# kai0511/insider

Measured on AMD Instinct MI355X. Metric: outer-iterations/sec (masked INSIDER fit, 10000 x 50000, K=30), higher is better.
Workload: dtype f64

## Files before the change

insider_amd/csrc/insider_col_factored.hpp:

```cpp
#pragma once

namespace insider {

constexpr int CP_MAXSTEPS = 8;
constexpr int CP_MAXCELLS = 4096;

struct ColFacArgs {
    int p, K, c;
    size_t plane;
    const uint32_t *grp[CF_MAXC];
    const uint16_t *slev[CF_MAXC];
    int L[CF_MAXC + 1], off[CF_MAXC + 1];
    int nlater[CF_MAXC + 1];
    int later_plane[CF_MAXC][CF_MAXC];
    int tab_skip_lo, tab_skip_n;
    int tab_rows;
    const double *Astack;
    const double *Qheld;
    const double *RtR;
    const double *yy_all, *yy_train;
    double *stat;
    const uint8_t *cnt;
    int cnt_stride, cnt_off[CF_MAXC + 1], nsteps;
    const float *hn;
    int hn_stride, hn_off[CF_MAXC + 1];
    const double *zt;
    int zt_stride, zt_off[CF_MAXC + 1];
    int m, SLcat;
    int pos_cov[CF_MAXC];
};

template <int NB, bool PREMASKED = false>
__device__ __forceinline__ void cf_store(d4 (&acc)[NB][NB], double *tr, const ColFacArgs &a, int j, int lane,
                                         const double *rtr, const double (&qh)[NB], double ss)
{
    constexpr int KP = Geo<NB>::KP;
    const int g4 = lane >> 4, c16 = lane & 15;
    double *out = a.stat + (size_t)j * Geo<NB>::STAT;
    int blk = 0;
#pragma unroll
    for (int bi = 0; bi < NB; ++bi)
#pragma unroll
        for (int bj = 0; bj <= bi; ++bj, ++blk) {
#pragma unroll
            for (int r = 0; r < 4; ++r) tr[(g4 + 4 * r) * 17 + c16] = acc[bj][bi][r];
            wave_sync();
            d4 res;
#pragma unroll
            for (int r = 0; r < 4; ++r) {
                const int ra = 16 * bi + g4 + 4 * r, cb = 16 * bj + c16;
                res[r] = acc[bi][bj][r] + tr[c16 * 17 + g4 + 4 * r];
                if constexpr (PREMASKED) res[r] = rtr[ra * KP + cb] - res[r];
// ... 204 lines not shown
            for (int s = 0; s < 4; ++s)
                if (l0 + 4 * s < Lo) {
#pragma unroll
                    for (int bi = 0; bi < NB; ++bi)
#pragma unroll
                        for (int bj = 0; bj < NB; ++bj)
                            acc[bi][bj] = __builtin_amdgcn_mfma_f64_16x16x4f64(cur.av[s][bi], P[bj][s], acc[bi][bj], 0, 0, 0);
                }
        };
        PairBlk<NB> b0, b1;
        fetch(0, b0);
        for (int l0 = 0; l0 < Lo; l0 += 32) {
            if (l0 + 16 < Lo) fetch(l0 + 16, b1);
            compute(l0, b0);
            if (l0 + 16 < Lo) {
                if (l0 + 32 < Lo) fetch(l0 + 32, b0);
                compute(l0 + 16, b1);
            }
        }
    }
    cf_store<NB, true>(acc, tr, a, j, lane, rtr, qh, ss);
}

template <int NB, int WPB, int MAXS, bool ZC = false>
__global__ void __launch_bounds__(WPB * 64) k_col_paircnt4(ColFacArgs a, unsigned *__restrict__ ticket, unsigned ticket_base, int npart, int cap)
{
    static_assert(NB <= 2, "accumulators of the 4x4x4 form");
    constexpr int KP = Geo<NB>::KP;
    extern __shared__ double s_c4[];
    const int w = __builtin_amdgcn_readfirstlane(threadIdx.x >> 6), lane = threadIdx.x & 63;
    double *tr = s_c4 + (size_t)w * 16 * 17;
    double *rtr = s_c4 + (size_t)WPB * 16 * 17;
    double *tabs = rtr + KP * KP;
    double *rows = tabs + 4 * a.nsteps * KP;
    const int npos = a.c + (ZC ? 1 : 0);
    for (int i = threadIdx.x; i < KP * KP; i += WPB * 64) rtr[i] = (i / KP < a.K && i % KP < a.K) ? a.RtR[i] : 0.0;
    for (int i = threadIdx.x; i < 4 * a.nsteps * KP; i += WPB * 64) {
        const int r = i / KP, k = i % KP;
        const int q = r < a.tab_skip_lo ? r : r + a.tab_skip_n;
        tabs[i] = r < a.tab_rows ? a.Astack[(size_t)q * KP + k] : 0.0;
    }
    {
        int pb4 = 0;
        for (int t = 0; t < npos; ++t) {
            const int nq = (a.L[t] + 3) >> 2;
            const double *At = a.Astack + (size_t)a.off[t] * KP;
            for (int i = threadIdx.x; i < 4 * nq * KP; i += WPB * 64) {
                const int l = i / KP, k = i % KP;
                rows[((size_t)(pb4 + (l >> 2)) * NB + (k >> 4)) * 64 + (l & 3) * 16 + (k & 15)] = At[i];
            }
            pb4 += nq;
        }
        for (int i = threadIdx.x; i < 4 * KP; i += WPB * 64) rows[(size_t)pb4 * NB * 64 + i] = 0.0;
    }
    __syncthreads();
    const int g4 = lane >> 4, c16 = lane & 15;
    constexpr int bpl = MAXS <= 4 ? 4 : 8;
    double tb[MAXS][NB];
#pragma unroll
    for (int s = 0; s < MAXS; ++s)
#pragma unroll
        for (int bb = 0; bb < NB; ++bb) tb[s][bb] = s < a.nsteps ? tabs[(4 * s + g4) * KP + 16 * bb + c16] : 0.0;
    double tbz[NB];
#pragma unroll
    for (int bb = 0; bb < NB; ++bb) tbz[bb] = ZC ? a.Astack[(size_t)(a.SLcat + g4) * KP + 16 * bb + c16] : 0.0;
    const unsigned off_c = (unsigned)lane * (unsigned)bpl, off_h = (unsigned)g4 * 4u;
    const double *rl[4];
#pragma unroll
    for (int x = 0; x < 4; ++x) rl[x] = rows + g4 * 16 + ((c16 + 4 * x) & 15);
    struct Blk {
        uint32_t cw[2];
        float4 hn;
        double z;
    };
    const int part = blockIdx.x % npart;
    unsigned *tk = ticket + 32 * part;
    auto take = [&]() {
        unsigned v = 0;
        if (lane == 0) v = atomicAdd(tk, 1u);
        return (unsigned)__builtin_amdgcn_readfirstlane((int)v) - ticket_base;
    };
    for (unsigned cur = take(), nxt; cur < (unsigned)cap; cur = nxt) {
    nxt = take();
    const int j = (int)cur * npart + part;
    if (j >= a.p) continue;
    double qh[NB];
#pragma unroll
    for (int bb = 0; bb < NB; ++bb) qh[bb] = a.Qheld[(size_t)j * KP + 16 * bb + c16];
    const double ss = a.yy_all[j] - a.yy_train[j];
    double acc[NB][NB][4];
#pragma unroll
    for (int bi = 0; bi < NB; ++bi)
#pragma unroll
        for (int bj = 0; bj < NB; ++bj)
#pragma unroll
            for (int x = 0; x < 4; ++x) acc[bi][bj][x] = 0.0;
    const uint8_t *cj = a.cnt + (size_t)j * a.cnt_stride;
    const float *hj = a.hn + (size_t)j * a.hn_stride;
    const double *zj = ZC ? a.zt + (size_t)j * a.zt_stride : nullptr;
    int pb4 = 0;
    for (int t = 0; t < npos; ++t) {
        const int Lo = a.L[t];
        const bool cross = a.nlater[t] > 0;
        const uint8_t *ct = cj + a.cnt_off[t];
        const float *ht = hj + a.hn_off[t];
        const double *zt = ZC ? zj + a.zt_off[t] : nullptr;
        auto fetch = [&](int l0, Blk &b) {
            if constexpr (ZC) b.z = zt[(size_t)(l0 >> 4) * 64 + lane];
            b.cw[0] = b.cw[1] = 0;
            if (cross) {
                const uint32_t *src = reinterpret_cast<const uint32_t *>(ct + (size_t)(l0 >> 4) * 64 * bpl + off_c);
                b.cw[0] = src[0];
                if (bpl == 8) b.cw[1] = src[1];
            }
            b.hn = *reinterpret_cast<const float4 *>(ht + l0 + off_h);
        };
        const double *rp[4];
#pragma unroll
        for (int x = 0; x < 4; ++x) rp[x] = rl[x] + (size_t)pb4 * NB * 64;
        auto rows_of = [&](int s, double (&av)[4][NB]) {
#pragma unroll
            for (int x = 0; x < 4; ++x)
#pragma unroll
                for (int bi = 0; bi < NB; ++bi) av[x][bi] = rp[x][(s * NB + bi) * 64];
        };
        auto step = [&](const double (&av)[4][NB], double hn, const d4 (&P)[NB], int s) {
            double pr[NB];
#pragma unroll
            for (int bb = 0; bb < NB; ++bb) pr[bb] = fma(hn, av[0][bb], P[bb][s]);
#pragma unroll
            for (int bi = 0; bi < NB; ++bi)
#pragma unroll
                for (int bj = 0; bj < NB; ++bj)
#pragma unroll
                    for (int x = 0; x < 4; ++x)
                        acc[bi][bj][x] = __builtin_amdgcn_mfma_f64_4x4x4f64(av[x][bi], pr[bj], acc[bi][bj][x], 0, 0, 0);
        };
        double avA[4][NB], avB[4][NB];
        auto compute = [&](int l0, const Blk &cur) {
            d4 P[NB];
#pragma unroll
            for (int bb = 0; bb < NB; ++bb) P[bb] = d4{0.0, 0.0, 0.0, 0.0};
            if (cross) {
#pragma unroll
                for (int s = 0; s < MAXS; ++s)
                    if (s < a.nsteps) {
                        const double cv = (double)((cur.cw[s >> 2] >> (8 * (s & 3))) & 0xffu);
#pragma unroll
                        for (int bb = 0; bb < NB; ++bb)
                            P[bb] = __builtin_amdgcn_mfma_f64_16x16x4f64(cv, tb[s][bb], P[bb], 0, 0, 0);
                    }
            }
            if constexpr (ZC) {
#pragma unroll
                for (int bb = 0; bb < NB; ++bb) P[bb] = __builtin_amdgcn_mfma_f64_16x16x4f64(cur.z, tbz[bb], P[bb], 0, 0, 0);
            }
            rows_of(1, avB);
            __builtin_amdgcn_sched_barrier(0);
            step(avA, (double)cur.hn.x, P, 0);
            if (l0 + 4 < Lo) {
                rows_of(2, avA);
            __builtin_amdgcn_sched_barrier(0);
                step(avB, (double)cur.hn.y, P, 1);
                if (l0 + 8 < Lo) {
                    rows_of(3, avB);
// ... 26 lines not shown
        const int b = c16 >> 2, jj = c16 & 3;
        double *out = a.stat + (size_t)j * Geo<NB>::STAT;
        int blk = 0;
#pragma unroll
        for (int bi = 0; bi < NB; ++bi)
#pragma unroll
            for (int bj = 0; bj <= bi; ++bj, ++blk) {
#pragma unroll
                for (int x = 0; x < 4; ++x) tr[(4 * ((b + x) & 3) + g4) * 17 + 4 * b + jj] = acc[bi][bj][x];
                wave_sync();
                d4 res;
#pragma unroll
                for (int r = 0; r < 4; ++r) res[r] = tr[(g4 + 4 * r) * 17 + c16];
                wave_sync();
#pragma unroll
                for (int x = 0; x < 4; ++x) tr[(4 * ((b + x) & 3) + g4) * 17 + 4 * b + jj] = acc[bj][bi][x];
                wave_sync();
#pragma unroll
                for (int r = 0; r < 4; ++r) {
                    const int ra = 16 * bi + g4 + 4 * r, cb = 16 * bj + c16;
                    res[r] = rtr[ra * KP + cb] - (res[r] + tr[c16 * 17 + g4 + 4 * r]);
                }
                wave_sync();
                if (bi == NB - 1 && g4 == 3) {
                    const int col = 16 * bj + c16;
                    res[3] = col < a.K ? qh[bj] : (col == KP - 1 ? ss : 0.0);
                }
#pragma unroll
                for (int r = 0; r < 4; ++r) out[blk * 256 + (g4 + 4 * r) * 16 + c16] = res[r];
            }
    }
    }
}

__global__ void __launch_bounds__(256) k_zt_build(ColFacArgs a, const uint32_t *__restrict__ col_ptr, const int *__restrict__ col_idx,
                                                  const double *__restrict__ col_val, const int *__restrict__ lev,
                                                  const double *__restrict__ Zc, int n, double *__restrict__ zt,
                                                  double *__restrict__ xz , int xz_pitch,
                                                  const double *__restrict__ S_all, double *__restrict__ S_train )
{
    const int w = threadIdx.x >> 6, lane = threadIdx.x & 63;
    const int j = blockIdx.x * 4 + w;
    if (j >= a.p) return;
    const uint32_t eb = col_ptr[j], ee = col_ptr[j + 1];
    double *zo = zt + (size_t)j * a.zt_stride;
    for (int t = 0; t < a.c; ++t) {
        const int *lv = lev + (size_t)a.pos_cov[t] * n;
        for (int l = lane; l < a.L[t]; l += WAVE) {
            double s[4] = {0.0, 0.0, 0.0, 0.0};
            for (uint32_t e = eb; e < ee; ++e) {
                const int i = col_idx[e];
                if (i < n && lv[i] == l) {
#pragma unroll
                    for (int k = 0; k < 4; ++k)
                        if (k < a.m) s[k] += Zc[(size_t)k * n + i];
// ... 216 lines not shown
```

insider_amd/csrc/insider_hip.hip:

```cpp
#include "insider_kernels.hpp"
#include "insider_posthoc.hpp"
#include "insider_vardecomp.hpp"
#include "insider_sampdecomp.hpp"
#include "insider_levelscores.hpp"
#include "insider_factdecomp.hpp"
#include "insider_rescomp.hpp"
#include "insider_outliers.hpp"
#include "insider_neighbors.hpp"
#include "insider_coexpr.hpp"
#include "insider_enrich.hpp"
#include "insider_kmeans.hpp"
#include "insider_tsne.hpp"

#include <rccl/rccl.h>

#include <algorithm>
#include <chrono>
#include <cstdlib>
#include <cmath>
#include <cstdio>
#include <cstring>
#include <limits>
#include <memory>
#include <mutex>
// ... 186 lines not shown
    DevBuf<int> lev, lvl_off_d, members_all, lvl_ptr_all, lvl_count_all;
    std::vector<CovTables> cov;
    CovTables cont;
    DevBuf<double> Zc;
    DevBuf<int> one_count;
    DevBuf<int> ident_members;
    int max_chunks = 0, max_L = 0, max_items = 0;
    DevBuf<double> S, yy_train, yy_all;
    DevBuf<double> Strain;
    DevBuf<double> Sheld;
    double cnt_train = 0, cnt_test = 0;
    bool no_na = false;
    DevBuf<uint32_t> col_ptr, row_ptr;
    DevBuf<int> col_idx, row_idx;
    DevBuf<double> col_val, row_val;
    DevBuf<uint8_t> col_flag;
    uint64_t col_entries = 0, row_entries = 0;
    bool merged = false;
    ColFacArgs cf;
    int cf_pos[CF_MAXC] = {0};
    bool cf_pair_ok = false;
    DevBuf<uint8_t> cf_cnt;
    DevBuf<float> cf_hn;
    DevBuf<double> cf_zt;
    std::vector<CovTables> contm;
    CovTables contm_lists;
    DevBuf<double> cont_cnt;
    bool cont_merged = false;
    std::vector<DevBuf<double>> cont_pair;
    std::shared_ptr<const HostTables> host;
    mutable std::mutex fold_mu;
    mutable std::shared_ptr<const FoldIds> folds;
    std::shared_ptr<const FoldIds> get_folds() const { std::lock_guard<std::mutex> g(fold_mu); return folds; }
    size_t bytes_shared = 0, bytes_own = 0;

    struct Block { int rows, off; };
    int blocks() const { return c + (m > 0 ? 1 : 0); }
    Block block(int b) const { return b < c ? Block{n_levels[b], lvl_off[b]} : Block{m, SLcat}; }

    DataSet() = default;
    DataSet(const DataSet &) = delete;
    DataSet &operator=(const DataSet &) = delete;
    ~DataSet() { (void)hipSetDevice(device); }
};

struct Workspace {
// ... 71 lines not shown
    }
    int synchronize_sides() const
    {
        for (const Stream *s : {&side, &side2, &side3}) HIPCHECK(hipStreamSynchronize(*s));
        return INSIDER_OK;
    }
    void synchronize() const
    {
        for (const Stream *s : {&stream, &side, &side2, &side3}) if (*s) (void)hipStreamSynchronize(*s);
    }
};

struct Options {
    int max_sweeps = 1 << 24, order_mode = 0, profile = 0, verbose = 0, cd_variant = 0, force_allreduce = 0;
    int col_factored = 1;
    int row_counts = 1;
    int row_merged = 1;
    int row_gemm = 1;
    int wg_waves = 1024;
    int row_fused = 1;
    int mm_fast = 1;
    int mm_tiles = 0;
    int col_mfma4 = 1;
    int cd_pairs = 1;
    int list_fine = 1;
    int cd_cold_iters = 3, cd_pass_first = 64, cd_pass_ratio = 4;
    double resid_stage_mb = 256.0;
    double vd_stage_kb = 48.0;
    int sd_slabs = 0;
    int ls_slabs = 0;
    double ls_part_mb = 256.0;
    int glm_slabs = 0;
    int rc_slabs = 0;
};

struct PostWs {
    DevBuf<double> Ast, U, cp, part, stats, stage, gpart, gram, cpart, gsum, L, dinv, outs;
    DevBuf<int> nz, ints, info;
    DevBuf<double> vin, vtab, vrec;
    DevBuf<double> spart, srec;
    DevBuf<double> lcand, ltab, lpart, lcnt, lout;
    DevBuf<double> fwall, fprod, fbase, frec;
    DevBuf<double> rq, rcs, rz, rpart, rin, rout;
    DevBuf<double> ocs, oz;
    DevBuf<uint32_t> obits;
    DevBuf<int> ogcnt, oscnt, orows, ocols;
// ... 1 lines not shown
};

}

struct insider_hip_handle {
    std::shared_ptr<const DataSet> ds;
    Streams st;
    Options opt;
    Workspace ws;
    PostWs post;
    FitPlan plan;
    bool w_ready = false;
    int64_t gene_offset = 0;
    int rank = 0, world = 1;
    insider_allreduce_fn allreduce = nullptr;
    void *allreduce_user = nullptr;
    ncclComm_t comm = nullptr;
    std::vector<Event> ev_col, ev_row, ev_cd, ev_test;
    double prof[12] = {0, 0, 0, 0, 0, 0, 0, 0, 0, 0, 0, 0};
    double steady_cd_ms = 0, steady_col_ms = 0;
    int cap_hits = 0, max_gene_sweeps = 0;
    int col_solver = 0, col_eval = 0, col_ridge_fallback = 0;
    int col_stats_kernel = 0, col_stats_tickets = 0, col_stats_blocks = 0;
    int col_q_kernel = 0, mm_rows2_tiles = 0;
    uint64_t row_kernels = 0;
    int vd_path = 0;
    int sd_path = 0, sd_slabs = 0;
    int ls_path = 0, ls_slabs = 0;
    int glm_slabs = 0, glm_form = 0;
    int fd_path = 0;
    int ls_form = 0, fd_form = 0, rc_form = 0, cx_form = 0;
    int rc_slabs = 0;
    double rc_ms = 0.0;
    double cx_stage_mb = 0.0, cx_stage_ms = 0.0, cx_ms = 0.0;
    int ol_path = 0;

    ~insider_hip_handle()
    {
        if (ds) (void)hipSetDevice(ds->device);
        st.synchronize();
        if (comm) (void)ncclCommDestroy(comm);
    }
};

namespace {

enum RowKernel {
    RK_WGEMM4 = 0, RK_WGEMM5, RK_WGEMM6, RK_WGEMM7, RK_WGEMM_CHUNKS, RK_WSYRK, RK_GRAM_SIDE,
    RK_GENE_U_CNT, RK_GENE_U, RK_GENE_UC,
    RK_MERGED_SOLVE, RK_MERGED, RK_MERGED_ZERO, RK_PACK_REDUCE,
    RK_LIST_STATS4, RK_LIST_STATS, RK_LEVEL_PARTIAL, RK_LEVEL_SOLVE, RK_CONT_CD,
    RK_MM_ROWS2, RK_MM_ROWS, RK_MM_REDUCE2_2, RK_MM_REDUCE2_4, RK_MM_REDUCE
};
inline uint64_t rk_bit(RowKernel k) { return 1ull << (int)k; }
inline void row_mark(insider_hip_handle *h, RowKernel k) { h->row_kernels |= rk_bit(k); }

PlanFacts plan_facts(const insider_hip_handle *h, int K)
{
    const DataSet &d = *h->ds;
    PlanFacts f;
    const Options &o = h->opt;
    f.opt = {o.row_merged, o.col_factored, o.row_fused, o.row_gemm, o.row_counts, o.mm_fast, o.force_allreduce, o.wg_waves,
             o.list_fine, o.mm_tiles, o.col_mfma4, o.cd_variant, o.cd_pairs, o.cd_cold_iters, o.cd_pass_first, o.cd_pass_ratio, o.max_sweeps};
    f.world = h->world; f.n_simd = d.n_simd;
    f.K = K; f.NB = h->ws.NB; f.KP = h->ws.KP; f.lvl_zero = (bool)h->ws.lvl_zero; f.fperm = (bool)h->ws.fperm;
    f.merged = d.merged; f.cont_merged = d.cont_merged; f.cf_pair_ok = d.cf_pair_ok; f.cf_hn = (bool)d.cf_hn; f.cf_zt = (bool)d.cf_zt;
    f.c = d.c; f.m = d.m; f.SL = d.SL; f.SLP = d.SLP; f.SLcat = d.SLcat; f.n = d.n; f.p = d.p; f.col_entries = d.col_entries; f.row_entries = d.row_entries;
    for (const CovTables &ct : d.cov) { f.L.push_back(ct.L); f.npairs.push_back(ct.npairs); }
    f.cf_c = d.cf.c; f.cf_tab_rows = d.cf.tab_rows; f.cf_nsteps = d.cf.nsteps;
    std::copy(d.cf.L, d.cf.L + CF_MAXC + 1, f.cf_L);
    std::copy(d.cf.nlater, d.cf.nlater + CF_MAXC + 1, f.cf_nlater);
    return f;
}

int ensure_workspace(insider_hip_handle *h, int K)
{
    if (K < 1 || K > INSIDER_MAX_K) return fail(INSIDER_ERR_UNSUPPORTED, "K must be in 1..63");
    if (h->ws.K == K) return INSIDER_OK;
    h->ws = Workspace();
    const DataSet &d = *h->ds;
    const hipStream_t st = h->st.stream;
    Workspace w;
    const int NB = (K + 1 + 15) / 16, KP = 16 * NB, NBLK = NB * (NB + 1) / 2, STAT = NBLK * 256;
    w.NB = NB;
    w.KP = KP;
    const int64_t avg_batches = (int64_t)(d.row_entries / (uint64_t)LIST_ALIGN / (uint64_t)std::max<int64_t>(d.n, 1));
    int nseg = (int)std::min<int64_t>(std::max<int64_t>(1, cdiv(8192, d.n)), std::max<int64_t>(1, avg_batches / 16));
    nseg = std::min(nseg, 64);
    w.nseg = nseg;
// ... 217 lines not shown
        HIPCHECK(hipFuncSetAttribute(reinterpret_cast<const void *>(&k_cd_cols_r16<3>), hipFuncAttributeMaxDynamicSharedMemorySize, lim));
        done.fetch_or(bit);
    }
    return INSIDER_OK;
}

int launch_gram(insider_hip_handle *h, const double *F, int64_t rows, double *out, hipStream_t st = nullptr,
                double *part = nullptr)
{
    return launch_mm_reduce_kp(h, F, h->ws.KP, F, (int)rows, h->ws.KP, part ? part : h->ws.gram_part, out, st);
}

int launch_build_R(insider_hip_handle *h)
{
    hipLaunchKernelGGL(k_build_R, dim3(cdiv(h->ds->n * h->ws.KP, 256)), dim3(256), 0, h->st.stream, (const int *)h->ds->lev,
                       (const int *)h->ds->lvl_off_d, h->ds->c, (int)h->ds->n, (const double *)h->ws.Astack, h->ws.KP,
                       (const double *)h->ds->Zc, h->ds->m, h->ds->SLcat, h->ws.R);
    KCHECK();
    return INSIDER_OK;
}

int phase_R(insider_hip_handle *h, bool use_side = false, bool r_is_current = false, bool want_qheld = false)
{
    if (use_side) {
        HIPCHECK(hipEventRecord(h->st.ev_a_ready, h->st.stream));
        HIPCHECK(hipStreamWaitEvent(h->st.side, h->st.ev_a_ready, 0));
        if (want_qheld && h->ws.Qheld && h->plan.col_path != 0) {
            HIPCHECK(hipStreamWaitEvent(h->st.side3, h->st.ev_a_ready, 0));
            if (int rh = launch_q(h, h->ds->Sheld, h->ws.Qheld, h->st.side3)) return rh;
            if (int rh = h->st.qheld.record(h->st.side3)) return rh;
        }
        int rq = launch_q(h, h->ds->S, h->ws.Qfull, h->st.side);
        if (rq) return rq;
        if ((rq = h->st.qfull.record(h->st.side))) return rq;
    }
    int rc = r_is_current ? INSIDER_OK : launch_build_R(h);
    if (rc) return rc;
    rc = launch_gram(h, h->ws.R, h->ds->n, h->ws.RtR);
    if (rc) return rc;
    if (use_side) return INSIDER_OK;
    return launch_q(h, h->ds->S, h->ws.Qfull);
}

struct Timer {
    Event e0, e1;
    int begin(insider_hip_handle *h, bool on)
    {
        if (!on || !h->opt.profile) return INSIDER_OK;
        HIPCHECK(hipEventCreateWithFlags(e0.out(), hipEventDisableSystemFence));
        HIPCHECK(hipEventCreateWithFlags(e1.out(), hipEventDisableSystemFence));
        HIPCHECK(hipEventRecord(e0, h->st.stream));
        return INSIDER_OK;
    }
    int end(insider_hip_handle *h, std::vector<Event> &into)
    {
        if (!e0) return INSIDER_OK;
        HIPCHECK(hipEventRecord(e1, h->st.stream));
        into.push_back(std::move(e0));
        into.push_back(std::move(e1));
        return INSIDER_OK;
    }
};

// ... 125 lines not shown
        hipLaunchKernelGGL(k_sched_bucket, dim3(cdiv(h->ds->p, 256)), dim3(256), 0, st, sweeps, (int)h->ds->p, reset, float_bits,
                           h->ws.sweep_key, cnt, h->ws.sched_bkt, h->ws.sched_rank);
    KCHECK();
    hipLaunchKernelGGL(k_sched_scatter, dim3(cdiv(h->ds->p, 256)), dim3(256), 0, st, (const int *)cnt, cnt_next,
                       (const uint16_t *)h->ws.sched_bkt, (const int *)h->ws.sched_rank, (int)h->ds->p, h->ws.gene_perm);
    KCHECK();
    return INSIDER_OK;
}

int launch_paircnt(insider_hip_handle *h, const ColFacArgs &a)
{
    const FitPlan &plan = h->plan;
    const size_t lds = plan.pc_lds;
    switch (plan.pc_kernel) {
        case CSK_PAIRCNT4_MS4:
        case CSK_PAIRCNT4_MS8:
        case CSK_PAIRCNT4_MS4_ZT: {
            const int nb = plan.pc_blocks, npart = plan.pc_parts, cap = cdiv(a.p, npart);
            const int which = npart == 1 ? 1 : 0;
            unsigned *tk = h->ws.pc4_ticket + (size_t)which * PC4_PARTS * 32;
            const unsigned tbase = h->ws.pc4_base[which];
#define PC4(NBV, MS)                                                                                                         \
    {                                                                                                                        \
        if (a.zt) hipLaunchKernelGGL((k_col_paircnt4<NBV, 4, MS, true>), dim3(nb), dim3(256), lds, h->st.stream, a, tk, tbase, npart, cap); \
        else hipLaunchKernelGGL((k_col_paircnt4<NBV, 4, MS, false>), dim3(nb), dim3(256), lds, h->st.stream, a, tk, tbase, npart, cap); \
    }
            const bool ms4 = plan.pc_kernel != CSK_PAIRCNT4_MS8;
            if (h->ws.NB == 1 && ms4) PC4(1, 4)
            else if (h->ws.NB == 1) PC4(1, 8)
            else if (ms4) PC4(2, 4)
            else PC4(2, 8)
#undef PC4
            KCHECK();
            h->ws.pc4_base[which] += (unsigned)cap + 4u * (unsigned)(nb / npart);
            h->col_stats_kernel = a.zt ? CSK_PAIRCNT4_MS4_ZT : ms4 ? CSK_PAIRCNT4_MS4 : CSK_PAIRCNT4_MS8;
            h->col_stats_tickets = npart;
            h->col_stats_blocks = nb;
            return INSIDER_OK;
        }
        case CSK_PAIRCNT:
        case CSK_PAIRCNT_ZT:
            NB_DISPATCH(h->ws.NB, {
                (void)WPB_;
                if (a.zt) hipLaunchKernelGGL((k_col_paircnt<NB_, 4, true>), dim3(cdiv(a.p, 4)), dim3(256), lds, h->st.stream, a);
                else hipLaunchKernelGGL((k_col_paircnt<NB_, 4, false>), dim3(cdiv(a.p, 4)), dim3(256), lds, h->st.stream, a);
            });
            KCHECK();
            h->col_stats_kernel = a.zt ? CSK_PAIRCNT_ZT : CSK_PAIRCNT;
            h->col_stats_tickets = h->col_stats_blocks = 0;
            return INSIDER_OK;
        default: return fail(INSIDER_ERR_ARG, "the call's plan names no pair-count statistics kernel");
    }
}

int launch_col_stats(insider_hip_handle *h, bool timed)
{
    Timer t;
    int rc;
    const bool factored = h->plan.col_path != 0;
    if (factored && h->st.qheld.pending) {
        if ((rc = h->st.qheld.wait(h->st.stream))) return rc;
        if ((rc = t.begin(h, timed))) return rc;
    } else {
        if ((rc = t.begin(h, timed))) return rc;
        if (factored)
            if ((rc = launch_q(h, h->ds->Sheld, h->ws.Qheld))) return rc;
    }
    if (factored) {
        ColFacArgs a = h->ds->cf;
        a.K = h->ws.K;
        a.Astack = h->ws.Astack;
        a.Qheld = h->ws.Qheld;
        a.RtR = h->ws.RtR;
        a.yy_all = h->ds->yy_all;
        a.yy_train = h->ds->yy_train;
        a.stat = h->ws.stat_col;
        if (h->plan.col_path == 2) {
            a.cnt = h->ds->cf_cnt;
            a.hn = h->ds->cf_hn;
            a.zt = h->ds->cf_zt;
            rc = launch_paircnt(h, a);
            if (rc) return rc;
        } else {
            NB_DISPATCH(h->ws.NB, {
                (void)WPB_;
                const size_t lds = ((size_t)(a.tab_rows + 1) * Geo<NB_>::KP + (size_t)4 * 16 * 17) * sizeof(double) + (size_t)4 * CF_CAP * 2;
                hipLaunchKernelGGL((k_col_factored<NB_, 4>), dim3(cdiv(h->ds->p, 4)), dim3(256), lds, h->st.stream, a);
            });
            h->col_stats_kernel = CSK_FACTORED;
            h->col_stats_tickets = h->col_stats_blocks = 0;
        }
        KCHECK();
    } else {
        uint64_t mark = 0;
        rc = launch_list_stats(h, true, 1, h->ws.R, h->ws.stat_col, h->ws.RtR, &mark);
        if (rc) return rc;
        h->col_stats_kernel = (mark & rk_bit(RK_LIST_STATS4)) ? CSK_LIST4 : CSK_LIST;
        h->col_stats_tickets = h->col_stats_blocks = 0;
    }
    return t.end(h, h->ev_col);
}

template <typename Args>
void col_args_head(const insider_hip_handle *h, int masked, int checkpoint, Args &a)
{
    a.stat = masked ? h->ws.stat_col : nullptr;
    a.stat_len = h->plan.stat_len;
    a.p = (int)h->ds->p;
    a.K = h->ws.K;
    a.KP = h->ws.KP;
    a.RtR = h->ws.RtR;
    a.Qfull = h->ws.Qfull;
    a.C = h->ws.C;
    a.yy = masked ? h->ds->yy_train : h->ds->yy_all;
    a.checkpoint = checkpoint;
    a.sse_train = h->ws.sse_train;
    a.b2 = h->ws.b2;
    a.b1 = h->ws.b1;
    a.sse_test = h->ws.sse_test;
    a.test_from_stats = masked && h->ds->no_na;
}

// ... 985 lines not shown
    if (fits && off <= 64 * 1024 && (size_t)p * (size_t)off <= ((size_t)1 << 32)) {
        if (off > 0) {
            DevBuf<int> ovf;
            if ((rc = d.cf_cnt.alloc((size_t)p * off)) || (rc = ovf.alloc(1))) return rc;
            HIPCHECK(hipMemsetAsync(ovf, 0, sizeof(int), st));
            hipLaunchKernelGGL((k_pair_count_build<2>), dim3(cdiv(p, 2)), dim3(128), 0, st, cf, d.cf_cnt, ovf);
            KCHECK();
            int hv = 0;
            HIPCHECK(hipMemcpyAsync(&hv, ovf, sizeof(int), hipMemcpyDeviceToHost, st));
            HIPCHECK(hipStreamSynchronize(st));
            fits = hv == 0;
        }
        if (fits && n < ((int64_t)1 << 24)) {
            int hoff = 0;
            for (int t = 0; t < c; ++t) {
                cf.hn_off[t] = hoff;
                hoff += ((cf.L[t] + 15) / 16) * 16;
            }
            cf.hn_stride = hoff;
            if ((rc = d.cf_hn.alloc((size_t)(p + 4) * hoff))) return rc;
            HIPCHECK(hipMemsetAsync(d.cf_hn, 0, (size_t)(p + 4) * hoff * sizeof(float), st));
            hipLaunchKernelGGL(k_half_counts, dim3((unsigned)cdiv((int64_t)p * hoff, 256)), dim3(256), 0, st, cf, d.cf_hn);
            KCHECK();
        } else {
            fits = false;
        }
        d.cf_pair_ok = fits;
    }
    cf.zt = nullptr;
    cf.m = d.m;
    cf.SLcat = d.SLcat;
    for (int t = 0; t < c; ++t) cf.pos_cov[t] = ord[t];
    return INSIDER_OK;
}

int stage_cont_factored(DataSet &d, hipStream_t st)
{
    const int64_t n = d.n, p = d.p;
    const int c = d.c, m = d.m;
    bool gu_fits = true;
    for (int t = 0; t < c; ++t)
        gu_fits = gu_fits && (size_t)4 * (d.SL + round_up(d.n_levels[t], 2) + GU_BATCH * WAVE) * sizeof(double) <= 64 * 1024;
    if (!(m > 0 && d.cf_pair_ok && gu_fits)) return INSIDER_OK;
    ColFacArgs &cf = d.cf;
    cf.L[c] = m;
    cf.off[c] = d.SLcat;
// ... 258 lines not shown
    if (!h || !name) return fail(INSIDER_ERR_ARG, "null");
    const std::string s(name);
    if (s == "max_sweeps") h->opt.max_sweeps = value < 1 ? 1 : (int)value;
    else if (s == "order_mode") h->opt.order_mode = (int)value;
    else if (s == "profile") h->opt.profile = (int)value;
    else if (s == "verbose") h->opt.verbose = (int)value;
    else if (s == "force_allreduce") h->opt.force_allreduce = (int)value;
    else if (s == "col_factored") h->opt.col_factored = (int)value;
    else if (s == "row_counts") h->opt.row_counts = (int)value;
    else if (s == "row_merged") h->opt.row_merged = (int)value;
    else if (s == "row_gemm_waves") {
        h->opt.wg_waves = std::max(64, (int)value);
        HIPCHECK(hipSetDevice(h->ds->device));
        h->ws = Workspace();
    }
    else if (s == "row_gemm") h->opt.row_gemm = (int)value;
    else if (s == "row_fused") h->opt.row_fused = (int)value;
    else if (s == "cd_cold_iters") h->opt.cd_cold_iters = (int)value;
    else if (s == "cd_pass1") h->opt.cd_pass_first = (int)value;
    else if (s == "cd_pass_ratio") h->opt.cd_pass_ratio = (int)value;
    else if (s == "list_fine") h->opt.list_fine = (int)value;
    else if (s == "mm_fast") h->opt.mm_fast = (int)value;
    else if (s == "mm_tiles") h->opt.mm_tiles = value < 1 ? 0 : (int)value;
    else if (s == "col_mfma4") h->opt.col_mfma4 = (int)value;
    else if (s == "cd_pairs") h->opt.cd_pairs = (int)value;
    else if (s == "resid_stage_mb") h->opt.resid_stage_mb = value;
    else if (s == "vd_stage_kb") h->opt.vd_stage_kb = value;
    else if (s == "ls_slabs") h->opt.ls_slabs = value < 1 ? 0 : (int)std::min(value, 256.0);
    else if (s == "rc_slabs") h->opt.rc_slabs = value < 1 ? 0 : (int)std::min(value, 256.0);
    else if (s == "ls_part_mb") h->opt.ls_part_mb = value;
    else if (s == "glm_slabs") h->opt.glm_slabs = value < 1 ? 0 : (int)std::min(value, 64.0);
    else if (s == "sd_slabs") h->opt.sd_slabs = value < 1 ? 0 : (int)std::min(value, 256.0);
    else if (s == "cd_variant") h->opt.cd_variant = (int)value;
    else return fail(INSIDER_ERR_ARG, "unknown option " + s);
    return INSIDER_OK;
}

static void reset_call_state(insider_hip_handle *h, bool drain)
{
    if (drain) (void)hipSetDevice(h->ds->device);
    if (drain) h->st.synchronize();
    h->w_ready = false;
    for (Join *j : {&h->st.qfull, &h->st.qheld, &h->st.side_done}) j->drop();
    clear_events(h);
}

// ... 1240 lines not shown
{
    if (!h || !name || !out) return fail(INSIDER_ERR_ARG, "null");
    const std::string s(name);
    const int NB = h->ws.NB;
    if (s == "col_stats_path") *out = build_plan(plan_facts(h, h->ws.K), 1).col_path;
    else if (s == "row_merged") *out = build_plan(plan_facts(h, h->ws.K), 1).merged ? 1.0 : 0.0;
    else if (s == "col_entries") *out = (double)h->ds->col_entries;
    else if (s == "row_entries") *out = (double)h->ds->row_entries;
    else if (s == "data_bytes_shared") *out = (double)h->ds->bytes_shared;
    else if (s == "data_bytes_own") *out = (double)h->ds->bytes_own;
    else if (s == "stat_doubles") *out = NB ? NB * (NB + 1) / 2 * 256.0 : 0.0;
    else if (s == "kp") *out = h->ws.KP;
    else if (s == "pair_count_bytes_per_gene") *out = h->ds->cf_pair_ok ? h->ds->cf.cnt_stride : 0.0;
    else if (s == "lists_bytes") *out = 12.0 * ((double)h->ds->col_entries + (double)h->ds->row_entries);
    else if (s == "cap_hits") *out = h->cap_hits;
    else if (s == "max_gene_sweeps") *out = h->max_gene_sweeps;
    else if (s == "max_sweeps") *out = h->opt.max_sweeps;
    else if (s == "col_solver") *out = h->col_solver;
    else if (s == "col_eval") *out = h->col_eval;
    else if (s == "col_ridge_fallback") *out = h->col_ridge_fallback;
    else if (s == "col_stats_kernel") *out = h->col_stats_kernel;
    else if (s == "col_stats_tickets") *out = h->col_stats_tickets;
    else if (s == "col_stats_blocks") *out = h->col_stats_blocks;
    else if (s == "col_q_kernel") *out = h->col_q_kernel;
    else if (s == "mm_rows2_tiles") *out = h->mm_rows2_tiles;
    else if (s == "n_simd") *out = h->ds->n_simd;
    else if (s == "row_kernels") *out = (double)h->row_kernels;
    else if (s == "cd_ms_steady") *out = h->steady_cd_ms;
    else if (s == "col_stats_ms_steady") *out = h->steady_col_ms;
    else if (s == "ol_path") *out = h->ol_path;
    else if (s == "vd_path") *out = h->vd_path;
    else if (s == "sd_path") *out = h->sd_path;
    else if (s == "ls_path") *out = h->ls_path;
    else if (s == "ls_slabs") *out = h->ls_slabs;
    else if (s == "sd_slabs") *out = h->sd_slabs;
    else if (s == "glm_slabs") *out = h->glm_slabs;
    else if (s == "glm_form") *out = h->glm_form;
    else if (s == "ls_form") *out = h->ls_form;
    else if (s == "fd_form") *out = h->fd_form;
    else if (s == "rc_form") *out = h->rc_form;
    else if (s == "cx_form") *out = h->cx_form;
    else if (s == "rc_slabs") *out = h->rc_slabs;
    else if (s == "cx_stage_mb") *out = h->cx_stage_mb;
    else if (s == "cx_stage_ms") *out = h->cx_stage_ms;
    else if (s == "cx_ms") *out = h->cx_ms;
    else if (s == "rc_ms") *out = h->rc_ms;
// ... 833 lines not shown
```

insider_amd/csrc/insider_plan.hpp:

```cpp
#pragma once

#include <algorithm>
#include <cmath>
#include <cstddef>
#include <cstdint>
#include <vector>

#include "insider_shapes.hpp"

namespace {

using namespace insider;

inline int64_t round_up(int64_t v, int64_t m) { return (v + m - 1) / m * m; }
inline int cdiv(int64_t a, int64_t b) { return (int)((a + b - 1) / b); }

enum ColSolver {
    CS_NONE = 0, CS_RIDGE_REG = 1, CS_RIDGE = 2, CS_CD_REG = 3, CS_CD_REG3 = 4, CS_CD_COLS16 = 5, CS_CD_COLS32 = 6,
    CS_CD_COLS64 = 7, CS_CD_R16_1 = 8, CS_CD_R16_2 = 9, CS_CD_R16_3 = 10
};

enum ColStatsKernel {
    CSK_NONE = 0, CSK_LIST = 1, CSK_LIST4 = 2, CSK_FACTORED = 3, CSK_PAIRCNT = 4, CSK_PAIRCNT_ZT = 5, CSK_PAIRCNT4_MS4 = 6,
    CSK_PAIRCNT4_MS8 = 7, CSK_PAIRCNT4_MS4_ZT = 8
};

enum ReduceForm { MR_REDUCE = 0, MR_REDUCE2_2 = 2, MR_REDUCE2_4 = 4 };

struct WgPlan {
    bool use = false;
    int tiles = 0, LT = 0, zch = 0, ntile = 0, npair = 0, slab = 0, nslab = 0;
};

struct PlanFacts {
    struct {
        int row_merged, col_factored, row_fused, row_gemm, row_counts, mm_fast, force_allreduce, wg_waves;
        int list_fine, mm_tiles, col_mfma4, cd_variant, cd_pairs, cd_cold_iters, cd_pass_first, cd_pass_ratio, max_sweeps;
    } opt{};
    int world = 1, n_simd = 1024;
    int K = 0, NB = 0, KP = 0;
    bool lvl_zero = false;
    bool fperm = false;
    bool merged = false, cont_merged = false, cf_pair_ok = false, cf_hn = false, cf_zt = false;
    int c = 0, m = 0, SL = 0, SLP = 0, SLcat = 0;
    int64_t n = 0, p = 0;
    uint64_t col_entries = 0, row_entries = 0;
    std::vector<int> L;
    std::vector<int64_t> npairs;
    int cf_c = 0, cf_tab_rows = 0, cf_nsteps = 0, cf_L[CF_MAXC + 1] = {0}, cf_nlater[CF_MAXC + 1] = {0};
};

struct ColCall {
    double alpha, la;
};

struct FitPlan {
    bool masked = false;
    bool merged = false;
    bool unmasked_fused = false;
    bool fused_solve = false;
    bool row_fused = false;
    bool allreduce = false;
    bool list4 = false;
    int mm_fast = 0;
    bool q_rows2 = false;
    bool v_rows2 = false;
    int mm_tpw = 1;
    int col_path = 0;
    int NB = 0, KP = 0, stat_len = 0, plen = 0;
    std::vector<WgPlan> wg;
    std::vector<uint8_t> u_cnt;
    ColStatsKernel pc_kernel = CSK_NONE;
    size_t pc_lds = 0;
    int pc_blocks = 0, pc_parts = 0;
    ColSolver col_solver = CS_NONE, col_eval = CS_NONE;
    bool ridge_fallback = false;
    int cold_iters = 0, npass = 0, pass_limit[16] = {0};
    bool order_wide = false, order_pairs = false;
};


inline bool list_stats4(const PlanFacts &f)
{
    const int NT = (f.K + 4) / 4;
    return f.opt.list_fine && f.NB == 2 && NT >= 5 && NT <= 8 && f.fperm;
}

inline int mm_tiles_per_wave(const PlanFacts &f, int tiles)
{
    if (f.opt.mm_tiles >= 1) return f.opt.mm_tiles;
    return std::max(1, tiles / (2 * f.n_simd));
}

inline bool mm_rows2_fits(const PlanFacts &f, int64_t ldx, int64_t M, int Kd)
{
    return f.opt.mm_fast && M >= MM_FAST_MIN && ldx % 2 == 0 && (size_t)4 * cdiv(Kd, 16) * f.NB * 64 * sizeof(double) <= 64 * 1024;
}
// ... 6 lines not shown
    return (cdiv(L, 16) <= 2 || p.mm_fast == 2 || p.NB > 2) ? MR_REDUCE2_2 : MR_REDUCE2_4;
}

inline void paircnt_plan(const PlanFacts &f, FitPlan &p)
{
    const int blocks = cdiv(f.p, 4), KP = f.KP, nsteps = f.cf_nsteps;
    const bool zt = f.cf_zt;
    if (f.opt.col_mfma4 && f.NB <= 2 && !(zt && nsteps > 4)) {
        size_t quads = 1;
        for (int t = 0; t < f.cf_c + (zt ? 1 : 0); ++t) quads += (size_t)(f.cf_L[t] + 3) / 4;
        const size_t lds = ((size_t)4 * 16 * 17 + (size_t)KP * KP + (size_t)4 * nsteps * KP + 4 * quads * KP) * sizeof(double);
        if (lds <= 64 * 1024) {
            const int resident = std::max(1, std::min((int)(160 * 1024 / lds), 3)) * std::max(1, f.n_simd / 4);
            int nb = std::min(blocks, resident);
            p.pc_parts = nb >= PC4_PARTS ? PC4_PARTS : 1;
            p.pc_blocks = nb - nb % p.pc_parts;
            p.pc_lds = lds;
            p.pc_kernel = zt ? CSK_PAIRCNT4_MS4_ZT : nsteps <= 4 ? CSK_PAIRCNT4_MS4 : CSK_PAIRCNT4_MS8;
            return;
        }
    }
    p.pc_lds = ((size_t)4 * 16 * 17 + (size_t)KP * KP + (size_t)4 * nsteps * KP) * sizeof(double);
    p.pc_kernel = zt ? CSK_PAIRCNT_ZT : CSK_PAIRCNT;
}

inline bool reg3_path(int K, double la) { return K > 32 && K <= 48 && la > 0.0; }

inline ColSolver cd_solver(int K, double la, int cd_variant)
{
    if (cd_variant == 0 && (K <= 32 || reg3_path(K, la)) && la > 0.0) return K <= 32 ? CS_CD_REG : CS_CD_REG3;
    if (cd_variant == 2 && K <= 16) return CS_CD_R16_1;
    if (cd_variant == 2 && K <= 32) return CS_CD_R16_2;
    if (K <= 16) return CS_CD_COLS16;
    if (K <= 32) return CS_CD_COLS32;
    if (cd_variant != 1 && K <= 48) return CS_CD_R16_3;
    return CS_CD_COLS64;
}

inline bool order_wide_rows(int K, ColSolver s) { return K > 32 && s != CS_CD_REG3; }

inline void col_solve_plan(const PlanFacts &f, const ColCall &c, FitPlan &p)
{
    const bool ridge = c.alpha == 0.0;
    p.col_solver = !ridge ? cd_solver(f.K, c.la, f.opt.cd_variant) : (f.K <= 32 && f.opt.cd_variant == 0) ? CS_RIDGE_REG : CS_RIDGE;
    p.ridge_fallback = p.col_solver == CS_RIDGE_REG;
    p.col_eval = p.col_solver == CS_CD_REG ? CS_CD_REG : p.col_solver == CS_CD_REG3 ? CS_CD_R16_3 : CS_NONE;
// ... 62 lines not shown
    double merged_us = 0.0;
    for (int i = 0; i < f.c; ++i)
        merged_us += (double)f.npairs[i] * mf * 1.1 + E * (f.c - 1) * 1.3e-6 + 33.0 * pscale * f.SLcat / 110.0 / f.c +
                     37.0 * pscale * f.L[i] / 100.0 + 40.0;
    return 1.1 * merged_us < old_us;
}

FitPlan build_plan(const PlanFacts &f, int masked, const ColCall *col = nullptr)
{
    FitPlan p;
    p.masked = masked != 0;
    p.merged = use_merged(f, masked);
    p.unmasked_fused = !masked && f.merged && f.opt.row_merged && f.opt.row_fused && f.m == 0 && f.lvl_zero;
    p.fused_solve = (p.merged || p.unmasked_fused) && f.world <= 1 && !f.opt.force_allreduce && f.opt.row_fused && f.NB <= 2;
    p.row_fused = f.opt.row_fused != 0;
    p.allreduce = f.world > 1 || f.opt.force_allreduce;
    p.list4 = list_stats4(f);
    p.mm_fast = f.opt.mm_fast;
    p.q_rows2 = mm_rows2_fits(f, f.SLP, f.p, f.SL);
    p.v_rows2 = f.opt.mm_fast && f.p >= MM_FAST_MIN;
    p.mm_tpw = mm_tiles_per_wave(f, cdiv(f.p, 16));
    p.col_path = col_stats_path(f);
    if (p.col_path == 2) paircnt_plan(f, p);
    if (col) col_solve_plan(f, *col, p);
    p.order_pairs = f.opt.cd_pairs && reg_pairs(reg_kmax(f.K));
    p.NB = f.NB;
    p.KP = f.KP;
    p.stat_len = f.NB * (f.NB + 1) / 2 * 256;
    p.plen = p.stat_len + 2 * f.KP + 2;
    for (int i = 0; i < f.c; ++i) {
        p.wg.push_back(wgemm_plan(f, i));
        const size_t gu_lds = (size_t)4 * (f.SL + round_up(f.L[i], 2) + GU_BATCH * WAVE) * sizeof(double);
        p.u_cnt.push_back(f.cf_pair_ok && (f.opt.row_counts || f.m > 0) && f.c <= CF_MAXC && gu_lds <= 64 * 1024);
    }
    return p;
}

}
```

insider_amd/csrc/insider_shapes.hpp:

```cpp
#pragma once

#include "../../include/insider_perm.h"

#if defined(__HIPCC__)
#define INSIDER_SHAPE_FN __host__ __device__ constexpr
#else
#define INSIDER_SHAPE_FN constexpr
#endif

namespace insider {

constexpr int WAVE = 64;

constexpr int CF_MAXC = 8;
constexpr int CF_CAP = 2048;
constexpr int GU_BATCH = 8;
constexpr int PC4_PARTS = 16;

constexpr int MM_SLAB = 128;
constexpr int MM_FAST_MIN = 16384;

INSIDER_SHAPE_FN bool reg_pairs(int KMAX) { return KMAX <= 30; }
INSIDER_SHAPE_FN int reg_kmax(int K) { return K <= 16 ? 16 : (K <= 32 ? (K + 1) & ~1 : (K + 3) & ~3); }

}
```

Baseline: 685.3.

## Fold Q and held-out Q products into the pair-count stats kernel

Adds a precomputed per-gene table of S and Sheld values, laid out per 16-level block, so the 4x4x4 pair-count stats kernel can fold those values into the padding columns of its products. The kernel then produces Qfull and Qheld itself. This removes the separate launch_q and side-stream Qheld GEMMs, along with the event synchronisation before the col stats, when the fit is masked, has no continuous covariates, and K leaves two spare padding columns. The cost is a larger persistent table, extra loads per block in the stats kernel, and a forced MAXS=4 instantiation.

New measurement: 705.8 (median of 6 runs). 1.03x the previous value.

```diff
diff --git a/insider_amd/csrc/insider_col_factored.hpp b/insider_amd/csrc/insider_col_factored.hpp
--- a/insider_amd/csrc/insider_col_factored.hpp
+++ b/insider_amd/csrc/insider_col_factored.hpp
@@ -28,6 +28,9 @@
     int zt_stride, zt_off[CF_MAXC + 1];
     int m, SLcat;
     int pos_cov[CF_MAXC];
+    const double *sq;
+    int sq_stride;
+    double *Qfull_out;
 };
 
 template <int NB, bool PREMASKED = false>
@@ -278,10 +281,11 @@
     cf_store<NB, true>(acc, tr, a, j, lane, rtr, qh, ss);
 }
 
-template <int NB, int WPB, int MAXS, bool ZC = false>
+template <int NB, int WPB, int MAXS, bool ZC = false, bool OWNQ = false>
 __global__ void __launch_bounds__(WPB * 64) k_col_paircnt4(ColFacArgs a, unsigned *__restrict__ ticket, unsigned ticket_base, int npart, int cap)
 {
     static_assert(NB <= 2, "accumulators of the 4x4x4 form");
+    static_assert(!(ZC && OWNQ), "continuous covariates keep the products over the genes");
     constexpr int KP = Geo<NB>::KP;
     extern __shared__ double s_c4[];
     const int w = __builtin_amdgcn_readfirstlane(threadIdx.x >> 6), lane = threadIdx.x & 63;
@@ -328,7 +332,9 @@
         uint32_t cw[2];
         float4 hn;
         double z;
+        double2 sq[2];
     };
+    const unsigned off_q = c16 == 14 ? g4 * 4u : c16 == 15 ? 16u + g4 * 4u : 32u;
     const int part = blockIdx.x % npart;
     unsigned *tk = ticket + 32 * part;
     auto take = [&]() {
@@ -342,7 +348,7 @@
     if (j >= a.p) continue;
     double qh[NB];
 #pragma unroll
-    for (int bb = 0; bb < NB; ++bb) qh[bb] = a.Qheld[(size_t)j * KP + 16 * bb + c16];
+    for (int bb = 0; bb < NB; ++bb) qh[bb] = OWNQ ? 0.0 : a.Qheld[(size_t)j * KP + 16 * bb + c16];
     const double ss = a.yy_all[j] - a.yy_train[j];
     double acc[NB][NB][4];
 #pragma unroll
@@ -354,6 +360,7 @@
     const uint8_t *cj = a.cnt + (size_t)j * a.cnt_stride;
     const float *hj = a.hn + (size_t)j * a.hn_stride;
     const double *zj = ZC ? a.zt + (size_t)j * a.zt_stride : nullptr;
+    const double *qj = OWNQ ? a.sq + (size_t)j * a.sq_stride + off_q : nullptr;
     int pb4 = 0;
     for (int t = 0; t < npos; ++t) {
         const int Lo = a.L[t];
@@ -361,6 +368,7 @@
         const uint8_t *ct = cj + a.cnt_off[t];
         const float *ht = hj + a.hn_off[t];
         const double *zt = ZC ? zj + a.zt_off[t] : nullptr;
+        const double *qt = OWNQ ? qj + (size_t)(a.hn_off[t] >> 4) * CF_SQ_BLOCK : nullptr;
         auto fetch = [&](int l0, Blk &b) {
             if constexpr (ZC) b.z = zt[(size_t)(l0 >> 4) * 64 + lane];
             b.cw[0] = b.cw[1] = 0;
@@ -370,6 +378,11 @@
                 if (bpl == 8) b.cw[1] = src[1];
             }
             b.hn = *reinterpret_cast<const float4 *>(ht + l0 + off_h);
+            if constexpr (OWNQ) {
+                const double2 *src = reinterpret_cast<const double2 *>(qt + (size_t)(l0 >> 4) * CF_SQ_BLOCK);
+                b.sq[0] = src[0];
+                b.sq[1] = src[1];
+            }
         };
         const double *rp[4];
 #pragma unroll
@@ -397,6 +410,7 @@
             d4 P[NB];
 #pragma unroll
             for (int bb = 0; bb < NB; ++bb) P[bb] = d4{0.0, 0.0, 0.0, 0.0};
+            if constexpr (OWNQ) P[NB - 1] = d4{cur.sq[0].x, cur.sq[0].y, cur.sq[1].x, cur.sq[1].y};
             if (cross) {
 #pragma unroll
                 for (int s = 0; s < MAXS; ++s)
@@ -469,15 +483,40 @@
                     res[r] = rtr[ra * KP + cb] - (res[r] + tr[c16 * 17 + g4 + 4 * r]);
                 }
                 wave_sync();
+                if constexpr (OWNQ) {
+                    if (bi == NB - 1 && bj == NB - 1 && c16 >= 14) res = d4{0.0, 0.0, 0.0, 0.0};
+                }
                 if (bi == NB - 1 && g4 == 3) {
                     const int col = 16 * bj + c16;
-                    res[3] = col < a.K ? qh[bj] : (col == KP - 1 ? ss : 0.0);
+                    res[3] = col < a.K ? (OWNQ ? -res[3] : qh[bj]) : (col == KP - 1 ? ss : 0.0);
+                }
+                if constexpr (OWNQ) {
+                    if (bi == NB - 1 && g4 == 2) {
+                        const int col = 16 * bj + c16;
+                        a.Qfull_out[(size_t)j * KP + col] = col < a.K ? -res[3] : 0.0;
+                        res[3] = 0.0;
+                    }
                 }
 #pragma unroll
                 for (int r = 0; r < 4; ++r) out[blk * 256 + (g4 + 4 * r) * 16 + c16] = res[r];
             }
     }
     }
+}
+
+__global__ void __launch_bounds__(256) k_own_q_table(ColFacArgs a, const double *__restrict__ S, const double *__restrict__ Sheld,
+                                                     int SLP, double *__restrict__ out)
+{
+    const size_t i = (size_t)blockIdx.x * blockDim.x + threadIdx.x;
+    if (i >= (size_t)a.p * a.sq_stride) return;
+    const int j = (int)(i / a.sq_stride), r = (int)(i % a.sq_stride);
+    const int blk = r / CF_SQ_BLOCK, x = r % CF_SQ_BLOCK;
+    int t = 0;
+    while (t + 1 < a.c && 16 * blk >= a.hn_off[t + 1]) ++t;
+    const int l = 16 * blk - a.hn_off[t] + 4 * (x & 3) + ((x >> 2) & 3);
+    double v = 0.0;
+    if (x < 32 && l < a.L[t]) v = (x < 16 ? S : Sheld)[(size_t)j * SLP + a.off[t] + l];
+    out[i] = v;
 }
 
 __global__ void __launch_bounds__(256) k_zt_build(ColFacArgs a, const uint32_t *__restrict__ col_ptr, const int *__restrict__ col_idx,
diff --git a/insider_amd/csrc/insider_hip.hip b/insider_amd/csrc/insider_hip.hip
--- a/insider_amd/csrc/insider_hip.hip
+++ b/insider_amd/csrc/insider_hip.hip
@@ -232,6 +232,7 @@
     bool cf_pair_ok = false;
     DevBuf<uint8_t> cf_cnt;
     DevBuf<float> cf_hn;
+    DevBuf<double> cf_sq;
     DevBuf<double> cf_zt;
     std::vector<CovTables> contm;
     CovTables contm_lists;
@@ -349,6 +350,7 @@
     int mm_fast = 1;
     int mm_tiles = 0;
     int col_mfma4 = 1;
+    int stats_own_q = 1;
     int cd_pairs = 1;
     int list_fine = 1;
     int cd_cold_iters = 3, cd_pass_first = 64, cd_pass_ratio = 4;
@@ -396,6 +398,7 @@
     int cap_hits = 0, max_gene_sweeps = 0;
     int col_solver = 0, col_eval = 0, col_ridge_fallback = 0;
     int col_stats_kernel = 0, col_stats_tickets = 0, col_stats_blocks = 0;
+    int col_stats_own_q = 0;
     int col_q_kernel = 0, mm_rows2_tiles = 0;
     uint64_t row_kernels = 0;
     int vd_path = 0;
@@ -435,10 +438,11 @@
     PlanFacts f;
     const Options &o = h->opt;
     f.opt = {o.row_merged, o.col_factored, o.row_fused, o.row_gemm, o.row_counts, o.mm_fast, o.force_allreduce, o.wg_waves,
-             o.list_fine, o.mm_tiles, o.col_mfma4, o.cd_variant, o.cd_pairs, o.cd_cold_iters, o.cd_pass_first, o.cd_pass_ratio, o.max_sweeps};
+             o.list_fine, o.mm_tiles, o.col_mfma4, o.cd_variant, o.cd_pairs, o.cd_cold_iters, o.cd_pass_first, o.cd_pass_ratio, o.max_sweeps,
+             o.stats_own_q};
     f.world = h->world; f.n_simd = d.n_simd;
     f.K = K; f.NB = h->ws.NB; f.KP = h->ws.KP; f.lvl_zero = (bool)h->ws.lvl_zero; f.fperm = (bool)h->ws.fperm;
-    f.merged = d.merged; f.cont_merged = d.cont_merged; f.cf_pair_ok = d.cf_pair_ok; f.cf_hn = (bool)d.cf_hn; f.cf_zt = (bool)d.cf_zt;
+    f.merged = d.merged; f.cont_merged = d.cont_merged; f.cf_pair_ok = d.cf_pair_ok; f.cf_hn = (bool)d.cf_hn; f.cf_zt = (bool)d.cf_zt; f.cf_sq = (bool)d.cf_sq;
     f.c = d.c; f.m = d.m; f.SL = d.SL; f.SLP = d.SLP; f.SLcat = d.SLcat; f.n = d.n; f.p = d.p; f.col_entries = d.col_entries; f.row_entries = d.row_entries;
     for (const CovTables &ct : d.cov) { f.L.push_back(ct.L); f.npairs.push_back(ct.npairs); }
     f.cf_c = d.cf.c; f.cf_tab_rows = d.cf.tab_rows; f.cf_nsteps = d.cf.nsteps;
@@ -702,7 +706,8 @@
 
 int phase_R(insider_hip_handle *h, bool use_side = false, bool r_is_current = false, bool want_qheld = false)
 {
-    if (use_side) {
+    const bool own_q = h->plan.stats_own_q;
+    if (use_side && !own_q) {
         HIPCHECK(hipEventRecord(h->st.ev_a_ready, h->st.stream));
         HIPCHECK(hipStreamWaitEvent(h->st.side, h->st.ev_a_ready, 0));
         if (want_qheld && h->ws.Qheld && h->plan.col_path != 0) {
@@ -718,7 +723,7 @@
     if (rc) return rc;
     rc = launch_gram(h, h->ws.R, h->ds->n, h->ws.RtR);
     if (rc) return rc;
-    if (use_side) return INSIDER_OK;
+    if (use_side || own_q) return INSIDER_OK;
     return launch_q(h, h->ds->S, h->ws.Qfull);
 }
 
@@ -890,7 +895,8 @@
             const unsigned tbase = h->ws.pc4_base[which];
 #define PC4(NBV, MS)                                                                                                         \
     {                                                                                                                        \
-        if (a.zt) hipLaunchKernelGGL((k_col_paircnt4<NBV, 4, MS, true>), dim3(nb), dim3(256), lds, h->st.stream, a, tk, tbase, npart, cap); \
+        if (plan.stats_own_q) hipLaunchKernelGGL((k_col_paircnt4<NBV, 4, 4, false, true>), dim3(nb), dim3(256), lds, h->st.stream, a, tk, tbase, npart, cap);  \
+        else if (a.zt) hipLaunchKernelGGL((k_col_paircnt4<NBV, 4, MS, true>), dim3(nb), dim3(256), lds, h->st.stream, a, tk, tbase, npart, cap); \
         else hipLaunchKernelGGL((k_col_paircnt4<NBV, 4, MS, false>), dim3(nb), dim3(256), lds, h->st.stream, a, tk, tbase, npart, cap); \
     }
             const bool ms4 = plan.pc_kernel != CSK_PAIRCNT4_MS8;
@@ -925,8 +931,10 @@
 {
     Timer t;
     int rc;
-    const bool factored = h->plan.col_path != 0;
-    if (factored && h->st.qheld.pending) {
+    const bool factored = h->plan.col_path != 0, own_q = h->plan.stats_own_q;
+    if (own_q) {
+        if ((rc = t.begin(h, timed))) return rc;
+    } else if (factored && h->st.qheld.pending) {
         if ((rc = h->st.qheld.wait(h->st.stream))) return rc;
         if ((rc = t.begin(h, timed))) return rc;
     } else {
@@ -939,6 +947,8 @@
         a.K = h->ws.K;
         a.Astack = h->ws.Astack;
         a.Qheld = h->ws.Qheld;
+        a.sq = own_q ? (const double *)h->ds->cf_sq : nullptr;
+        a.Qfull_out = own_q ? (double *)h->ws.Qfull : nullptr;
         a.RtR = h->ws.RtR;
         a.yy_all = h->ds->yy_all;
         a.yy_train = h->ds->yy_train;
@@ -966,6 +976,7 @@
         h->col_stats_kernel = (mark & rk_bit(RK_LIST_STATS4)) ? CSK_LIST4 : CSK_LIST;
         h->col_stats_tickets = h->col_stats_blocks = 0;
     }
+    h->col_stats_own_q = own_q ? 1 : 0;
     return t.end(h, h->ev_col);
 }
 
@@ -1997,6 +2008,13 @@
             HIPCHECK(hipMemsetAsync(d.cf_hn, 0, (size_t)(p + 4) * hoff * sizeof(float), st));
             hipLaunchKernelGGL(k_half_counts, dim3((unsigned)cdiv((int64_t)p * hoff, 256)), dim3(256), 0, st, cf, d.cf_hn);
             KCHECK();
+            cf.sq_stride = hoff / 16 * CF_SQ_BLOCK;
+            if (d.m == 0 && (int64_t)p * cf.sq_stride / 256 < ((int64_t)1 << 31)) {
+                if (d.cf_sq.alloc((size_t)p * cf.sq_stride)) { (void)hipGetLastError(); d.cf_sq.reset(); }
+                else hipLaunchKernelGGL(k_own_q_table, dim3((unsigned)cdiv((int64_t)p * cf.sq_stride, 256)), dim3(256), 0, st, cf,
+                                   (const double *)d.S, (const double *)d.Sheld, (int)d.SLP, (double *)d.cf_sq);
+                KCHECK();
+            }
         } else {
             fits = false;
         }
@@ -2301,6 +2319,7 @@
     else if (s == "list_fine") h->opt.list_fine = (int)value;
     else if (s == "mm_fast") h->opt.mm_fast = (int)value;
     else if (s == "mm_tiles") h->opt.mm_tiles = value < 1 ? 0 : (int)value;
+    else if (s == "stats_own_q") h->opt.stats_own_q = (int)value;
     else if (s == "col_mfma4") h->opt.col_mfma4 = (int)value;
     else if (s == "cd_pairs") h->opt.cd_pairs = (int)value;
     else if (s == "resid_stage_mb") h->opt.resid_stage_mb = value;
@@ -3587,6 +3606,7 @@
     else if (s == "col_stats_kernel") *out = h->col_stats_kernel;
     else if (s == "col_stats_tickets") *out = h->col_stats_tickets;
     else if (s == "col_stats_blocks") *out = h->col_stats_blocks;
+    else if (s == "col_stats_own_q") *out = h->col_stats_own_q;
     else if (s == "col_q_kernel") *out = h->col_q_kernel;
     else if (s == "mm_rows2_tiles") *out = h->mm_rows2_tiles;
     else if (s == "n_simd") *out = h->ds->n_simd;
diff --git a/insider_amd/csrc/insider_plan.hpp b/insider_amd/csrc/insider_plan.hpp
--- a/insider_amd/csrc/insider_plan.hpp
+++ b/insider_amd/csrc/insider_plan.hpp
@@ -36,12 +36,13 @@
     struct {
         int row_merged, col_factored, row_fused, row_gemm, row_counts, mm_fast, force_allreduce, wg_waves;
         int list_fine, mm_tiles, col_mfma4, cd_variant, cd_pairs, cd_cold_iters, cd_pass_first, cd_pass_ratio, max_sweeps;
+        int stats_own_q;
     } opt{};
     int world = 1, n_simd = 1024;
     int K = 0, NB = 0, KP = 0;
     bool lvl_zero = false;
     bool fperm = false;
-    bool merged = false, cont_merged = false, cf_pair_ok = false, cf_hn = false, cf_zt = false;
+    bool merged = false, cont_merged = false, cf_pair_ok = false, cf_hn = false, cf_zt = false, cf_sq = false;
     int c = 0, m = 0, SL = 0, SLP = 0, SLcat = 0;
     int64_t n = 0, p = 0;
     uint64_t col_entries = 0, row_entries = 0;
@@ -73,6 +74,7 @@
     ColStatsKernel pc_kernel = CSK_NONE;
     size_t pc_lds = 0;
     int pc_blocks = 0, pc_parts = 0;
+    bool stats_own_q = false;
     ColSolver col_solver = CS_NONE, col_eval = CS_NONE;
     bool ridge_fallback = false;
     int cold_iters = 0, npass = 0, pass_limit[16] = {0};
@@ -125,6 +127,13 @@
     }
     p.pc_lds = ((size_t)4 * 16 * 17 + (size_t)KP * KP + (size_t)4 * nsteps * KP) * sizeof(double);
     p.pc_kernel = zt ? CSK_PAIRCNT_ZT : CSK_PAIRCNT;
+}
+
+inline bool stats_own_q(const PlanFacts &f, const FitPlan &p, bool col_call)
+{
+    if (!(f.opt.stats_own_q >= 2 || (f.opt.stats_own_q == 1 && col_call))) return false;
+    if (!(p.masked && p.col_path == 2 && p.pc_kernel == CSK_PAIRCNT4_MS4)) return false;
+    return f.cf_sq && f.m == 0 && !f.cf_zt && f.world <= 1 && f.K <= f.KP - 2;
 }
 
 inline bool reg3_path(int K, double la) { return K > 32 && K <= 48 && la > 0.0; }
@@ -233,6 +242,7 @@
     p.mm_tpw = mm_tiles_per_wave(f, cdiv(f.p, 16));
     p.col_path = col_stats_path(f);
     if (p.col_path == 2) paircnt_plan(f, p);
+    p.stats_own_q = stats_own_q(f, p, col != nullptr);
     if (col) col_solve_plan(f, *col, p);
     p.order_pairs = f.opt.cd_pairs && reg_pairs(reg_kmax(f.K));
     p.NB = f.NB;
diff --git a/insider_amd/csrc/insider_shapes.hpp b/insider_amd/csrc/insider_shapes.hpp
--- a/insider_amd/csrc/insider_shapes.hpp
+++ b/insider_amd/csrc/insider_shapes.hpp
@@ -16,6 +16,7 @@
 constexpr int CF_CAP = 2048;
 constexpr int GU_BATCH = 8;
 constexpr int PC4_PARTS = 16;
+constexpr int CF_SQ_BLOCK = 36;
 
 constexpr int MM_SLAB = 128;
 constexpr int MM_FAST_MIN = 16384;
```
